# yu45020/Text_Segmentation_Image_Inpainting

Measured on NVIDIA H100. Metric: PartialConv UNet 512x512 images/sec (fwd+bwd), higher is better.
Workload: dtype bf16

## Files before the change

### text_segmentation_image_inpainting_b200/csrc/conv_tc.cu

```cuda
#include <cuda.h>
#include <stdlib.h>
#include <string.h>

#include <algorithm>

#include "pcb_common.cuh"
#include "pcb_ptx.cuh"

namespace {

constexpr int BLOCK_M = 128;
constexpr int BLOCK_K = 64;
constexpr int A_STAGE_BYTES = BLOCK_M * 128;
constexpr int NUM_PRODUCER_THREADS = 128;
constexpr int TC_MAX_PARTS = 2;
constexpr int MMA_WARPS = 8;
constexpr int MMA_THREADS = MMA_WARPS * 32;
constexpr int acc_pitch(int block_n) { return block_n + 4; }
constexpr int acc_stage_bytes(int block_n) { return BLOCK_M * acc_pitch(block_n) * 4; }

inline int rup(int v, int m) { return (v + m - 1) / m * m; }

struct TcPart {
    const bf16 *x;
// ... 7 lines not shown
    int n, h, w, cin, cout, kh, kw, stride, pad_h, pad_w, dil, ho, wo;
    int m_total;
    int nparts, no_guard, rowpack;
    int hg;
    int ring_a, ring_b;
    int ktap;
    int ncols;
    TcPart parts[TC_MAX_PARTS];
    const float *bias; const float *msum; bf16 *y; int y_cstride;
    const bf16 *dc; int dc_cstride, dc_c8, dc_kext;
    int *abort_flag;
    int l2pf;
    int box_w, box_h, box_n, stages, use_fix;
    int wk_base, wk_row, wk_col;
    int sub, py, px, fh, fw;
    int ksplit;
    float *partial;
    double *bn_sums;
    int bn_c;
};

constexpr int STAT_SLICE = 256;
constexpr int STAT_SMEM_BYTES = MMA_WARPS * STAT_SLICE * 4 + 16;

__device__ __forceinline__ float warp_transpose_sum(float (&v)[32], int lane) {
#pragma unroll
    for (int off = 16, n = 32; off >= 1; off >>= 1, n >>= 1) {
        const bool upper = (lane & off) != 0;
#pragma unroll
        for (int i = 0; i < 16; ++i) {
            if (i < (n >> 1)) {
                const float send = upper ? v[i] : v[i + (n >> 1)];
                const float keep = upper ? v[i + (n >> 1)] : v[i];
                v[i] = keep + __shfl_xor_sync(0xffffffffu, send, off);
            }
        }
    }
    return v[0];
}

__device__ __forceinline__ uint32_t align1024(uint32_t a) { return (a + 1023u) & ~1023u; }

__device__ __forceinline__ void load_acc32(const float *src, uint32_t (&r)[32]) {
#pragma unroll
    for (int j = 0; j < 8; ++j) {
        const uint4 v = reinterpret_cast<const uint4 *>(src)[j];
        r[4 * j] = v.x; r[4 * j + 1] = v.y; r[4 * j + 2] = v.z; r[4 * j + 3] = v.w;
    }
}

template <int BLOCK_N, int MODE>
__device__ __forceinline__ void tc_epilogue(const TcParams &P, const float *acc_row, int warp, int lane, int m0, int n0, float *s_stat,
                                            int cb, int ce, int sq_off) {
                const int row = warp * 32 + lane;
                const int m = m0 + row;
                const bool rvalid = m < P.m_total;
                float inv = 0.f;
                bool hole = false;
                int en = 0, eh = 0, ew = 0;
                long long mo = m;
                if (MODE == 1 && rvalid) {
                    en = m / (P.h * P.w); const int rem = m - en * P.h * P.w; eh = rem / P.w; ew = rem - eh * P.w;
                    eh = eh * P.sub + P.py; ew = ew * P.sub + P.px;
                    mo = (static_cast<long long>(en) * P.fh + eh) * P.fw + ew;
                }
                if (MODE == 0 && rvalid && P.sub != 1) {
                    en = m / (P.ho * P.wo); const int rem = m - en * P.ho * P.wo; eh = rem / P.wo; ew = rem - eh * P.wo;
                    mo = (static_cast<long long>(en) * P.fh + eh * P.sub + P.py) * P.fw + ew * P.sub + P.px;
                }
                if (MODE == 0 && rvalid) {
                    const float s = P.msum ? P.msum[mo] : 1.f;
                    hole = (s == 0.f) && !P.no_guard;
                    inv = hole ? 0.f : 1.0f / s;
                }
                if (P.partial != nullptr) {
    #pragma unroll 1
                    for (int c0 = cb; c0 < ce; c0 += 32) {
                        uint32_t r[32];
                        load_acc32(acc_row + c0, r);
                        if (rvalid) {
                            float *dst = P.partial + static_cast<long long>(m) * P.ncols + n0 + c0;
    #pragma unroll
                            for (int j = 0; j < 32; ++j) atomicAdd(dst + j, __uint_as_float(r[j]));
                        }
                    }
                    return;
                }
    #pragma unroll 1
                for (int c0 = cb; c0 < ce; c0 += 32) {
                    uint32_t r[32];
                    load_acc32(acc_row + c0, r);
                    const int col = n0 + c0;
                    bf16 *orow = nullptr;
                    int nstore = 0;
                    float scale = inv;
                    if (MODE == 0) {
                        if (rvalid && col < P.y_cstride) { orow = P.y + mo * P.y_cstride + col; nstore = min(32, P.y_cstride - col); }
                    } else {
                        scale = 1.f;
                        for (int p = 0; p < P.nparts; ++p) {
                            const TcPart &pt = P.parts[p];
                            const int local = col - pt.koff;
                            if (local >= 0 && local < pt.kext && pt.dx != nullptr && local < pt.c8 && rvalid) {
                                orow = pt.dx + mo * pt.dx_cstride + local;
                                nstore = min(32, pt.c8 - local);
                                if (pt.mask != nullptr)
                                    scale = pt.mask[(static_cast<long long>(en) * (P.fh >> pt.mup) + (eh >> pt.mup)) * (P.fw >> pt.mup) + (ew >> pt.mup)] ? 1.f : 0.f;
                            }
                        }
                    }
                    const bool stats = (MODE == 0) && (s_stat != nullptr);
                    if (__any_sync(0xffffffffu, nstore > 0) || stats) {
                        uint4 o[4];
                        __nv_bfloat162 *ob = reinterpret_cast<__nv_bfloat162 *>(o);
                        float bl = 0.f;
                        const bool has_bias = (MODE == 0) && (P.bias != nullptr);
                        if (has_bias && col + lane < P.cout) bl = P.bias[col + lane];
                        const bool edge = (MODE == 0) && (col + 32 > P.cout);
    #pragma unroll
                        for (int j = 0; j < 16; ++j) {
                            float a = __uint_as_float(r[2 * j]), b = __uint_as_float(r[2 * j + 1]);
                            if (MODE == 0) {
                                const float b0 = has_bias ? __shfl_sync(0xffffffffu, bl, 2 * j) : 0.f;
                                const float b1 = has_bias ? __shfl_sync(0xffffffffu, bl, 2 * j + 1) : 0.f;
                                a = hole ? 0.f : fmaf(a, scale, b0);
                                b = hole ? 0.f : fmaf(b, scale, b1);
                                if (edge) {
                                    if (col + 2 * j >= P.cout) a = 0.f;
                                    if (col + 2 * j + 1 >= P.cout) b = 0.f;
                                }
// ... 32 lines not shown
        const int co = n0 + c0 + lane;
        if (co < P.bn_c) {
            atomicAdd(P.bn_sums + co, static_cast<double>(s_stat[c0 - cb + lane]));
            atomicAdd(P.bn_sums + P.bn_c + co, static_cast<double>(s_stat[sq_off + c0 - cb + lane]));
        }
        s_stat[c0 - cb + lane] = 0.f; s_stat[sq_off + c0 - cb + lane] = 0.f;
    }
    __syncwarp();
}

template <int BLOCK_N>
struct EpiRole {
    static constexpr int HN = (BLOCK_N >= 64) ? BLOCK_N / 2 : BLOCK_N;
    int q, half, cb, ce;
    __device__ __forceinline__ explicit EpiRole(int e) {
        q = 2 * (e >> 2) + (e & 1);
        half = (e & 3) >> 1;
        cb = half * HN;
        ce = (cb + HN <= BLOCK_N) ? cb + HN : cb;
    }
    __device__ __forceinline__ int slice() const { return half * 4 + q; }
};

template <int BLOCK_N, int MODE>
__device__ __forceinline__ void mma_epilogue(const TcParams &P, const float (&acc)[BLOCK_N / 2], float *stage, int e, int lane, int m0, int n0,
                                             float *s_stat) {
    constexpr int PITCH = acc_pitch(BLOCK_N);
    const int g = e >> 2;
    const int r0 = 64 * g + 16 * (e & 3) + (lane >> 2), c0 = 2 * (lane & 3);
#pragma unroll
    for (int i = 0; i < BLOCK_N / 2; i += 2) {
        const int row = r0 + 8 * ((i >> 1) & 1), col = 8 * (i >> 2) + c0;
        *reinterpret_cast<float2 *>(stage + row * PITCH + col) = make_float2(acc[i], acc[i + 1]);
    }
    ptx::named_sync(1 + g, 128);
    const EpiRole<BLOCK_N> R(e);
    tc_epilogue<BLOCK_N, MODE>(P, stage + (R.q * 32 + lane) * PITCH, R.q, lane, m0, n0, s_stat, R.cb, R.ce, 128);
    ptx::named_sync(1 + g, 128);
}

template <int BLOCK_N>
__device__ __forceinline__ void tc_stats_final(const TcParams &P, const float *stat_base, int e, int lane, int stat_n0) {
    constexpr int HN = EpiRole<BLOCK_N>::HN;
    for (int col = e * 32 + lane; col < BLOCK_N; col += MMA_THREADS) {
        const int co = stat_n0 + col;
        if (co < P.bn_c) {
            const int h = col / HN, lc = col - h * HN;
            float a = 0.f, q = 0.f;
#pragma unroll
            for (int w4 = 0; w4 < 4; ++w4) { a += stat_base[(h * 4 + w4) * STAT_SLICE + lc]; q += stat_base[(h * 4 + w4) * STAT_SLICE + 128 + lc]; }
            atomicAdd(P.bn_sums + co, static_cast<double>(a));
            atomicAdd(P.bn_sums + P.bn_c + co, static_cast<double>(q));
        }
    }
}

template <int R> __device__ __forceinline__ void zero_acc(float (&a)[R]) {
#pragma unroll
    for (int i = 0; i < R; ++i) a[i] = 0.f;
}

constexpr int HALO_MAX_HG = 12;
constexpr int PERSIST_THREADS = 4 * 32 + MMA_THREADS + 32;
constexpr int MAX_RING = 8;

template <int BLOCK_N, int MODE, bool HALO>
__global__ void __launch_bounds__(PERSIST_THREADS, 1)
pconv_tc_persistent_kernel(const __grid_constant__ TcParams P, const __grid_constant__ CUtensorMap tmap_w) {
    constexpr int B_STAGE_BYTES = BLOCK_N * 128;
    extern __shared__ uint8_t smem_raw[];
    const uint32_t smem_base = align1024(ptx::smem_u32(smem_raw));
    const int SA = P.ring_a, SB = P.ring_b;
    const int HG = P.hg;
// ... 335 lines not shown
                    } else {
                        const uint64_t da = ptx::make_smem_desc(sA + sa * A_STAGE + g * a_rows, 16, 1024);
#pragma unroll
                        for (int k = 0; k < BLOCK_K / 16; ++k)
                            ptx::wgmma_bf16<BLOCK_N, 0, 0>(acc, da + 2 * k, db + 2 * k);
                    }
                    ptx::wgmma_commit();
                }
                ptx::wgmma_wait<0>();
                ptx::wgmma_fence_regs(acc);
                if (leader) {
                    for (int tc = 0; tc < nB; ++tc) ptx::mbar_arrive(bar_empty_b + 8 * ((sb0 + tc) % SB));
                    ptx::mbar_arrive(bar_empty_a + 8 * sa);
                }
            }
            if (dead) { stat_n0 = -1; break; }
            mma_epilogue<BLOCK_N, MODE>(P, acc, acc_stage, e, lane, m0, n0, my_stat);
        }
        if (my_stat && stat_n0 >= 0) tc_stats_flush<BLOCK_N>(P, my_stat, lane, stat_n0, R.cb, R.ce, 128);
    }
}


constexpr int TMA_THREADS = MMA_THREADS + 5 * 32;

template <int BLOCK_N, int MODE, bool HALO>
__global__ void __launch_bounds__(TMA_THREADS, 1)
pconv_tc_tma_kernel(const __grid_constant__ TcParams P, const __grid_constant__ CUtensorMap tmap_w,
                    const __grid_constant__ CUtensorMap tmap_a0, const __grid_constant__ CUtensorMap tmap_a1) {
    constexpr uint32_t B_BYTES = BLOCK_N * 128;
    extern __shared__ uint8_t smem_raw[];
    const uint32_t smem_base = align1024(ptx::smem_u32(smem_raw));
    const int S = P.stages;
    const int nB = HALO ? P.kw : 1;
    const int hx = HALO ? (P.kw - 1) * P.dil : 0;
    const uint32_t A_BYTES = static_cast<uint32_t>(BLOCK_M + hx) * 128u;
    const uint32_t A_ROOM = (A_BYTES + 1023u) & ~1023u;
    const uint32_t STAGE = A_ROOM + nB * B_BYTES;
    const uint32_t STAGE_TX = A_BYTES + nB * B_BYTES;
    const uint32_t sBar = smem_base + S * STAGE;
    const uint32_t bar_full = sBar, bar_fixed = sBar + 8 * MAX_RING, bar_empty = sBar + 16 * MAX_RING;
    const uint32_t s_stat_addr = sBar + 24 * MAX_RING;
    const uint32_t s_acc = (s_stat_addr + STAT_SMEM_BYTES + 15u) & ~15u;
    uint8_t *smem_gen = smem_raw + (smem_base - ptx::smem_u32(smem_raw));

    const int warp = __shfl_sync(0xffffffffu, threadIdx.x >> 5, 0), lane = threadIdx.x & 31;
    const int np = (MODE == 0) ? P.nparts : 1;
    const int n_tiles = P.ncols / BLOCK_N;
    const int KS = P.ksplit;
    const int m_tiles = (P.m_total + BLOCK_M - 1) / BLOCK_M;
    const int num_tiles = m_tiles * n_tiles * KS;
    const int tile0 = static_cast<int>(blockIdx.x), tstep = static_cast<int>(gridDim.x);
    auto m0_of = [&](int mt) -> int { return mt * BLOCK_M; };
    const bool fix = (MODE == 0) && P.use_fix;
    const int kwi = HALO ? 1 : P.kw;

    auto tile_active = [&](int n0) -> bool {
        if (MODE == 0) return true;
        for (int p = 0; p < P.nparts; ++p)
            if (P.parts[p].dx && n0 < P.parts[p].koff + P.parts[p].kext && n0 + BLOCK_N > P.parts[p].koff) return true;
        return false;
    };

    if (threadIdx.x == 0) {
        for (int s = 0; s < MAX_RING; ++s) {
            ptx::mbar_init(bar_full + 8 * s, 1); ptx::mbar_init(bar_fixed + 8 * s, 4); ptx::mbar_init(bar_empty + 8 * s, 2);
        }
        ptx::fence_mbar_init();
    }
    if (warp == 8 && lane == 0) { ptx::prefetch_tmap(&tmap_w); ptx::prefetch_tmap(&tmap_a0); if (np > 1) ptx::prefetch_tmap(&tmap_a1); }
    __syncthreads();

    float *s_stat = nullptr;
    int stat_n0 = -1;
    if (warp == 8) {
        int s = 0;
        uint32_t ph = 1;
        const int plane = (MODE == 0) ? P.ho * P.wo : P.h * P.w;
        const int pwid = (MODE == 0) ? P.wo : P.w;
        const int kext0 = (MODE == 0) ? P.parts[0].kext : P.dc_kext, kext1 = (MODE == 0 && np > 1) ? P.parts[1].kext : 0;
        const int dstep = (MODE == 0) ? P.dil : -P.dil;
        const int row_k = P.wk_row, col_k = P.wk_col;
        bool dead = false;
        for (int tile = tile0; tile < num_tiles && !dead; tile += tstep) {
            const int sp = tile % KS, mn = tile / KS;
            const int m0 = m0_of(mn / n_tiles), n0 = (mn % n_tiles) * BLOCK_N;
            if (!tile_active(n0)) continue;
            const int img = m0 / plane, rem = m0 - img * plane;
            const int oy = rem / pwid, ox = rem - oy * pwid;
            const int x_org = (MODE == 0) ? ox * P.stride - P.pad_w : (HALO ? ox + P.pad_w - hx : ox + P.pad_w);
            const int y_org = (MODE == 0) ? oy * P.stride - P.pad_h : oy + P.pad_h;
            int nx_org = 0, ny_org = 0, nimg = -1;
            if (P.l2pf && tile + tstep < num_tiles) {
                const int nmn = (tile + tstep) / KS;
                const int nm0 = m0_of(nmn / n_tiles);
                if (nm0 != m0) {
                    nimg = nm0 / plane;
                    const int nrem = nm0 - nimg * plane, noy = nrem / pwid, nox = nrem - noy * pwid;
// ... 24 lines not shown
                            __syncwarp();
                            if (++s == S) { s = 0; ph ^= 1; }
                        }
                        if (dead) break;
                    }
                }
        }
    } else if (warp < MMA_WARPS) {
        const int e = warp, g = warp >> 2;
        const bool leader = (threadIdx.x & 127) == 0;
        const uint32_t ready = fix ? bar_fixed : bar_full;
        const uint64_t desc_a0 = ptx::make_smem_desc(smem_base + g * 64 * 128, 16, 1024);
        const uint64_t desc_b0 = ptx::make_smem_desc(smem_base + A_ROOM, 16, 1024);
        const uint32_t stage16 = STAGE >> 4;
        const int shift0 = (HALO && MODE == 1) ? hx * 8 : 0;
        const int dshift = HALO ? ((MODE == 1) ? -P.dil * 8 : P.dil * 8) : 0;
        const int rows_a = P.kh * kwi;
        int nb0, nb1 = 0, kl0, kl1 = 4;
        {
            const int kext = (MODE == 0) ? P.parts[0].kext : P.dc_kext, c8 = (MODE == 0) ? P.parts[0].c8 : P.dc_c8;
            nb0 = kext / BLOCK_K; kl0 = min(4, (c8 - (nb0 - 1) * BLOCK_K + 15) >> 4);
            if (MODE == 0 && np > 1) { nb1 = P.parts[1].kext / BLOCK_K; kl1 = min(4, (P.parts[1].c8 - (nb1 - 1) * BLOCK_K + 15) >> 4); }
        }
        const EpiRole<BLOCK_N> R(e);
        s_stat = (MODE == 0 && P.bn_sums != nullptr && P.partial == nullptr)
                     ? reinterpret_cast<float *>(smem_gen + (s_stat_addr - smem_base)) + R.slice() * STAT_SLICE : nullptr;
        if (s_stat) {
            for (int i = lane; i < STAT_SLICE; i += 32) s_stat[i] = 0.f;
            __syncwarp();
        }
        float *acc_stage = reinterpret_cast<float *>(smem_gen + (s_acc - smem_base));
        int s = 0;
        uint32_t ph = 0;
        bool dead = false;
        for (int tile = tile0; tile < num_tiles && !dead; tile += tstep) {
            const int sp = tile % KS, mn = tile / KS;
            const int m0 = m0_of(mn / n_tiles), n0 = (mn % n_tiles) * BLOCK_N;
            if (!tile_active(n0)) continue;
            if (s_stat && n0 != stat_n0) {
                if (stat_n0 >= 0) tc_stats_flush<BLOCK_N>(P, s_stat, lane, stat_n0, R.cb, R.ce, 128);
                stat_n0 = n0;
            }
            float acc[BLOCK_N / 2];
            zero_acc(acc);
            int held = -1;
            for (int r = 0; r < rows_a && !dead; ++r) {
#pragma unroll
                for (int p = 0; p < TC_MAX_PARTS; ++p) {
                    const int nbp = (p == 0) ? nb0 : nb1, klast = (p == 0) ? kl0 : kl1;
                    const int gb0 = (p == 0) ? 0 : nb0;
                    for (int cb = 0; cb < nbp; ++cb) {
                        if (KS > 1 && (gb0 + cb) % KS != sp) continue;
                        if (!__all_sync(0xffffffffu, ptx::mbar_wait(ready + 8 * s, ph, P.abort_flag, 124))) { dead = true; break; }
                        uint64_t da = desc_a0 + static_cast<uint64_t>(s * stage16 + shift0), db = desc_b0 + static_cast<uint64_t>(s * stage16);
                        const int ksteps = (cb + 1 < nbp) ? 4 : klast;
                        ptx::wgmma_fence();
                        for (int tc = 0; tc < nB; ++tc, da += dshift, db += B_BYTES >> 4) {
                            if (ksteps == 4) {
#pragma unroll
                                for (int k = 0; k < 4; ++k) ptx::wgmma_bf16<BLOCK_N, 0, 0>(acc, da + 2 * k, db + 2 * k);
                            } else {
                                for (int k = 0; k < ksteps; ++k) ptx::wgmma_bf16<BLOCK_N, 0, 0>(acc, da + 2 * k, db + 2 * k);
                            }
                        }
                        ptx::wgmma_commit();
                        ptx::wgmma_wait<1>();
                        if (held >= 0 && leader) ptx::mbar_arrive(bar_empty + 8 * held);
                        held = s;
                        if (++s == S) { s = 0; ph ^= 1; }
                    }
                    if (dead) break;
                }
            }
            ptx::wgmma_wait<0>();
            ptx::wgmma_fence_regs(acc);
            if (held >= 0 && leader) ptx::mbar_arrive(bar_empty + 8 * held);
            if (dead) { stat_n0 = -1; break; }
            mma_epilogue<BLOCK_N, MODE>(P, acc, acc_stage, e, lane, m0, n0, s_stat);
        }
    } else if (warp > 8) {
        if (fix) {
            const int t = (warp - 9) * 32 + lane;
            int s = 0;
            uint32_t ph = 0;
            bool dead = false;
            if (!HALO) {
                uint64_t wnext[TC_MAX_PARTS];
                auto load_words = [&](int tl) {
#pragma unroll
                    for (int p = 0; p < TC_MAX_PARTS; ++p) {
                        wnext[p] = 0ull;
                        const int m = m0_of(tl / KS / n_tiles) + t;
                        if (fix && p < P.nparts && tl < num_tiles && m < P.m_total) wnext[p] = __ldg(P.parts[p].tapmask + m);
                    }
                };
                load_words(tile0);
                for (int tile = tile0; tile < num_tiles && !dead; tile += tstep) {
                    const int sp = tile % KS;
                    uint64_t wcur[TC_MAX_PARTS];
#pragma unroll
                    for (int p = 0; p < TC_MAX_PARTS; ++p) wcur[p] = wnext[p];
// ... 75 lines not shown
#pragma unroll
                                        for (int k = 0; k < 8; ++k) r[k] = z;
                                    }
                                    if (h1) {
                                        uint4 *r = reinterpret_cast<uint4 *>(smem_gen + s * STAGE + (t + 128) * 128);
#pragma unroll
                                        for (int k = 0; k < 8; ++k) r[k] = z;
                                    }
                                    ptx::fence_proxy_async_smem();
                                }
                                __syncwarp();
                                if (lane == 0) ptx::mbar_arrive(bar_fixed + 8 * s);
                                if (++s == S) { s = 0; ph ^= 1; }
                            }
                            if (dead) break;
                        }
                    }
                }
            }
        }
    }

    __syncthreads();
    if (s_stat != nullptr && stat_n0 >= 0) tc_stats_final<BLOCK_N>(P, s_stat - EpiRole<BLOCK_N>(warp).slice() * STAT_SLICE, warp, lane, stat_n0);
}


constexpr int SP_MAX_ITEMS = 40;
struct SpItem { int part, dx, dy, wk, nb, wk_step, shift0, dshift; };
struct SpTable {
    int n_items;
    int step[TC_MAX_PARTS];
    int es[TC_MAX_PARTS];
    int ph[TC_MAX_PARTS], pw[TC_MAX_PARTS];
    int arows[TC_MAX_PARTS];
    int rows_max;
    SpItem it[SP_MAX_ITEMS];
};

template <int BLOCK_N, int MODE>
__global__ void __launch_bounds__(TMA_THREADS, 1)
pconv_tc_sp_kernel(const __grid_constant__ TcParams P, const __grid_constant__ SpTable TB, const __grid_constant__ CUtensorMap tmap_w,
                   const __grid_constant__ CUtensorMap tmap_a0, const __grid_constant__ CUtensorMap tmap_a1) {
    constexpr uint32_t B_BYTES = BLOCK_N * 128;
    extern __shared__ uint8_t smem_raw[];
    const uint32_t smem_base = align1024(ptx::smem_u32(smem_raw));
    const int S = P.stages;
    int nb_max = 1;
    for (int i = 0; i < TB.n_items; ++i) nb_max = max(nb_max, TB.it[i].nb);
    const uint32_t A_ROOM = (static_cast<uint32_t>(TB.rows_max) * 128u + 1023u) & ~1023u;
    const uint32_t STAGE = A_ROOM + nb_max * B_BYTES;
    const uint32_t sBar = smem_base + S * STAGE;
    const uint32_t bar_full = sBar, bar_fixed = sBar + 8 * MAX_RING, bar_empty = sBar + 16 * MAX_RING;
    const uint32_t s_stat_addr = sBar + 24 * MAX_RING;
    const uint32_t s_acc = (s_stat_addr + STAT_SMEM_BYTES + 15u) & ~15u;
    uint8_t *smem_gen = smem_raw + (smem_base - ptx::smem_u32(smem_raw));

    const int warp = __shfl_sync(0xffffffffu, threadIdx.x >> 5, 0), lane = threadIdx.x & 31;
    const int n_tiles = P.ncols / BLOCK_N;
    const int m_tiles = (P.m_total + BLOCK_M - 1) / BLOCK_M;
    const int num_tiles = m_tiles * n_tiles;
    const int tile0 = static_cast<int>(blockIdx.x), tstep = static_cast<int>(gridDim.x);
    const bool fix = P.use_fix != 0;
    const int gw = (MODE == 0) ? P.wo : P.w, gh = (MODE == 0) ? P.ho : P.h;
    const int plane = gw * gh;
    int nbk[TC_MAX_PARTS], klast[TC_MAX_PARTS];
#pragma unroll
    for (int p = 0; p < TC_MAX_PARTS; ++p) {
        const int kext = (MODE == 0) ? P.parts[p].kext : P.dc_kext, c8 = (MODE == 0) ? P.parts[p].c8 : P.dc_c8;
        nbk[p] = (p < ((MODE == 0) ? P.nparts : 1)) ? kext / BLOCK_K : 0;
        klast[p] = nbk[p] ? min(4, (c8 - (nbk[p] - 1) * BLOCK_K + 15) >> 4) : 4;
    }

    if (threadIdx.x == 0) {
        for (int s = 0; s < MAX_RING; ++s) { ptx::mbar_init(bar_full + 8 * s, 1); ptx::mbar_init(bar_fixed + 8 * s, 4); ptx::mbar_init(bar_empty + 8 * s, 2); }
        ptx::fence_mbar_init();
    }
    if (warp == 8 && lane == 0) { ptx::prefetch_tmap(&tmap_w); ptx::prefetch_tmap(&tmap_a0); ptx::prefetch_tmap(&tmap_a1); }
    __syncthreads();

    float *s_stat = nullptr;
    int stat_n0 = -1;
    if (warp == 8) {
        int s = 0;
        uint32_t ph = 1;
        bool dead = false;
        for (int tile = tile0; tile < num_tiles && !dead; tile += tstep) {
            const int m0 = (tile / n_tiles) * BLOCK_M, n0 = (tile % n_tiles) * BLOCK_N;
            const int img = m0 / plane, rem = m0 - img * plane;
            const int oy = rem / gw, ox = rem - oy * gw;
            for (int i = 0; i < TB.n_items && !dead; ++i) {
                const SpItem it = TB.it[i];
                const CUtensorMap *ma = (it.part == 0) ? &tmap_a0 : &tmap_a1;
                const int x = ox * TB.step[it.part] + it.dx, y = oy * TB.step[it.part] + it.dy;
                const uint32_t a_bytes = static_cast<uint32_t>(TB.arows[it.part]) * 128u;
                for (int cb = 0; cb < nbk[it.part]; ++cb) {
                    if (!__all_sync(0xffffffffu, ptx::mbar_wait(bar_empty + 8 * s, ph, P.abort_flag, 321))) { dead = true; break; }
                    if (ptx::elect_one()) {
                        const uint32_t full = bar_full + 8 * s, dst = smem_base + s * STAGE;
                        ptx::mbar_arrive_expect_tx(full, a_bytes + it.nb * B_BYTES);
                        ptx::tma_load_4d(dst, ma, cb * BLOCK_K, x, y, img, full);
                        uint32_t bdst = dst + A_ROOM;
                        for (int tc = 0, kb = it.wk + cb * BLOCK_K; tc < it.nb; ++tc, kb += it.wk_step, bdst += B_BYTES)
                            ptx::tma_load_2d(bdst, &tmap_w, kb, n0, full);
                    }
                    __syncwarp();
                    if (++s == S) { s = 0; ph ^= 1; }
                }
            }
        }
    } else if (warp < MMA_WARPS) {
        const int e = warp, g = warp >> 2;
        const bool leader = (threadIdx.x & 127) == 0;
        const uint32_t ready = fix ? bar_fixed : bar_full;
        const uint64_t desc_a0 = ptx::make_smem_desc(smem_base + g * 64 * 128, 16, 1024);
        const uint64_t desc_b0 = ptx::make_smem_desc(smem_base + A_ROOM, 16, 1024);
        const uint32_t stage16 = STAGE >> 4;
        const EpiRole<BLOCK_N> R(e);
        s_stat = (MODE == 0 && P.bn_sums != nullptr) ? reinterpret_cast<float *>(smem_gen + (s_stat_addr - smem_base)) + R.slice() * STAT_SLICE : nullptr;
        if (s_stat) {
            for (int i = lane; i < STAT_SLICE; i += 32) s_stat[i] = 0.f;
            __syncwarp();
        }
        float *acc_stage = reinterpret_cast<float *>(smem_gen + (s_acc - smem_base));
        int s = 0;
        uint32_t ph = 0;
        bool dead = false;
        for (int tile = tile0; tile < num_tiles && !dead; tile += tstep) {
            const int m0 = (tile / n_tiles) * BLOCK_M, n0 = (tile % n_tiles) * BLOCK_N;
            if (s_stat && n0 != stat_n0) {
                if (stat_n0 >= 0) tc_stats_flush<BLOCK_N>(P, s_stat, lane, stat_n0, R.cb, R.ce, 128);
                stat_n0 = n0;
            }
            float acc[BLOCK_N / 2];
            zero_acc(acc);
            int held = -1;
            for (int i = 0; i < TB.n_items && !dead; ++i) {
                const SpItem it = TB.it[i];
                for (int cb = 0; cb < nbk[it.part]; ++cb) {
                    if (!__all_sync(0xffffffffu, ptx::mbar_wait(ready + 8 * s, ph, P.abort_flag, 324))) { dead = true; break; }
                    uint64_t da = desc_a0 + static_cast<uint64_t>(s * stage16 + it.shift0), db = desc_b0 + static_cast<uint64_t>(s * stage16);
                    const int ksteps = (cb + 1 < nbk[it.part]) ? 4 : klast[it.part];
                    ptx::wgmma_fence();
                    for (int tc = 0; tc < it.nb; ++tc, da += it.dshift, db += B_BYTES >> 4)
                        for (int k = 0; k < ksteps; ++k) ptx::wgmma_bf16<BLOCK_N, 0, 0>(acc, da + 2 * k, db + 2 * k);
                    ptx::wgmma_commit();
                    ptx::wgmma_wait<1>();
                    if (held >= 0 && leader) ptx::mbar_arrive(bar_empty + 8 * held);
                    held = s;
                    if (++s == S) { s = 0; ph ^= 1; }
                }
            }
            ptx::wgmma_wait<0>();
            ptx::wgmma_fence_regs(acc);
            if (held >= 0 && leader) ptx::mbar_arrive(bar_empty + 8 * held);
            if (dead) { stat_n0 = -1; break; }
            mma_epilogue<BLOCK_N, MODE>(P, acc, acc_stage, e, lane, m0, n0, s_stat);
        }
    } else if (warp > 8) {
        if (fix) {
            const int t = (warp - 9) * 32 + lane;
            int s = 0;
            uint32_t ph = 0;
            bool dead = false;
            auto load_bits = [&](int tl, uint64_t &b0, uint64_t &b1) {
                b0 = b1 = 0ull;
                if (tl >= num_tiles) return;
                const int m0 = (tl / n_tiles) * BLOCK_M;
                const int img = m0 / plane, rem = m0 - img * plane;
                const int oy = rem / gw, ox = rem - oy * gw;
                for (int i = 0; i < TB.n_items; ++i) {
                    const SpItem it = TB.it[i];
                    const uint8_t *mk = P.parts[it.part].mask;
                    if (mk == nullptr) continue;
                    const int pwid = TB.pw[it.part], phei = TB.ph[it.part], es = TB.es[it.part];
                    const int hrows = TB.arows[it.part] - BLOCK_M;
                    const int x0 = ox * TB.step[it.part] + it.dx, y0 = oy * TB.step[it.part] + it.dy;
                    int tx, ty, tn;
                    if (hrows > 0 || (P.box_h == 1 && P.box_n == 1)) { tx = t; ty = 0; tn = 0; }
                    else { tx = t % P.box_w; ty = (t / P.box_w) % P.box_h; tn = t / (P.box_w * P.box_h); }
// ... 21 lines not shown
                            const uint4 z = make_uint4(0u, 0u, 0u, 0u);
                            if (h0) {
                                uint4 *r = reinterpret_cast<uint4 *>(smem_gen + s * STAGE + t * 128);
#pragma unroll
                                for (int k = 0; k < 8; ++k) r[k] = z;
                            }
                            if (h1) {
                                uint4 *r = reinterpret_cast<uint4 *>(smem_gen + s * STAGE + (t + 128) * 128);
#pragma unroll
                                for (int k = 0; k < 8; ++k) r[k] = z;
                            }
                            ptx::fence_proxy_async_smem();
                        }
                        __syncwarp();
                        if (lane == 0) ptx::mbar_arrive(bar_fixed + 8 * s);
                        if (++s == S) { s = 0; ph ^= 1; }
                    }
                }
            }
        }
    }

    __syncthreads();
    if (s_stat != nullptr && stat_n0 >= 0) tc_stats_final<BLOCK_N>(P, s_stat - EpiRole<BLOCK_N>(warp).slice() * STAT_SLICE, warp, lane, stat_n0);
}

__global__ void upsample_part_kernel(const bf16 *__restrict__ src, int cstride, int c8, long long pixels_src, int hs, int ws, bf16 *__restrict__ dst) {
    const int chunks = c8 >> 3;
    const long long total = pixels_src * chunks;
    for (long long i = blockIdx.x * static_cast<long long>(blockDim.x) + threadIdx.x; i < total; i += static_cast<long long>(gridDim.x) * blockDim.x) {
        const int ch = static_cast<int>(i % chunks);
        const long long pix = i / chunks;
        const int x = static_cast<int>(pix % ws);
        const long long t = pix / ws;
        const int y = static_cast<int>(t % hs);
        const long long n = t / hs;
        const uint4 v = __ldg(reinterpret_cast<const uint4 *>(src + pix * cstride + ch * 8));
        bf16 *d = dst + ((n * (2 * hs) + 2 * y) * (2ll * ws) + 2 * x) * c8 + ch * 8;
        uint4 *d0 = reinterpret_cast<uint4 *>(d), *d1 = reinterpret_cast<uint4 *>(d + 2ll * ws * c8);
        d0[0] = v; *reinterpret_cast<uint4 *>(d + c8) = v;
        d1[0] = v; *reinterpret_cast<uint4 *>(d + 2ll * ws * c8 + c8) = v;
    }
}

struct WgParams {
    int n, h, w, cin, cout, kh, kw, stride, pad_h, pad_w, dil, ho, wo;
    int m_total;
// ... 780 lines not shown
}

bool tma_dgrad_s2_ok(const pcb_conv *c) {
    if (getenv("PCB_DISABLE_TMA") || getenv("PCB_DISABLE_TMA_S2") || is_rowpack(c)) return false;
    if (c->stride != 2 || c->dil != 1 || c->kh < 2 || c->kw < 2 || ((c->h | c->w) & 1) || c->ho != c->h / 2 || c->wo != c->w / 2) return false;
    int bw, bh, bn;
    return tile_box(c->w / 2, c->h / 2, &bw, &bh, &bn);
}

size_t up_bytes(const pcb_conv *c, int p) {
    return (static_cast<size_t>(c->n) * c->h * c->w * rup(c->parts[p].c, 8) * 2 + 255) / 256 * 256;
}
size_t tapmask_bytes(const pcb_conv *c) {
    return (static_cast<size_t>(c->nparts) * c->n * c->ho * c->wo * sizeof(uint64_t) + 255) / 256 * 256;
}

template <int BLOCK_N, int MODE, bool HALO>
int launch_tma_n(TcParams &P, const CUtensorMap &tw, const CUtensorMap &ta0, const CUtensorMap &ta1, cudaStream_t st) {
    const int nb = HALO ? P.kw : 1;
    const size_t a_room = (static_cast<size_t>(BLOCK_M + (HALO ? (P.kw - 1) * P.dil : 0)) * 128 + 1023) / 1024 * 1024;
    const size_t stage = a_room + static_cast<size_t>(nb) * BLOCK_N * 128;
    P.stages = static_cast<int>(std::min<size_t>(MAX_RING, (RING_BUDGET - acc_stage_bytes(BLOCK_N)) / stage));
    PCB_CHECK(P.stages >= 2, "TMA-fed conv: stage of %zu bytes does not fit twice", stage);
    const size_t smem = 1024 + P.stages * stage + 24 * MAX_RING + 16 + STAT_SMEM_BYTES + acc_stage_bytes(BLOCK_N);
    auto kern = pconv_tc_tma_kernel<BLOCK_N, MODE, HALO>;
    PCB_SMEM_OPT_IN(kern, MAX_SMEM);
    if (P.ksplit < 1) P.ksplit = 1;
    const int m_tiles = (P.m_total + BLOCK_M - 1) / BLOCK_M;
    const int num_tiles = m_tiles * (P.ncols / BLOCK_N) * P.ksplit;
    const int grid = std::min(num_tiles, pcb_num_sms());
    kern<<<grid, TMA_THREADS, smem, st>>>(P, tw, ta0, ta1);
    PCB_LAUNCH_CHECK();
    return 0;
}

template <int MODE>
int launch_tma(TcParams &P, const CUtensorMap &tw, const CUtensorMap &ta0, const CUtensorMap &ta1, int bn, bool halo, cudaStream_t st) {
    if (halo) {
        if (bn == 128) return launch_tma_n<128, MODE, true>(P, tw, ta0, ta1, st);
        if (bn == 64) return launch_tma_n<64, MODE, true>(P, tw, ta0, ta1, st);
        return launch_tma_n<32, MODE, true>(P, tw, ta0, ta1, st);
    }
    if (bn == 128) return launch_tma_n<128, MODE, false>(P, tw, ta0, ta1, st);
    if (bn == 64) return launch_tma_n<64, MODE, false>(P, tw, ta0, ta1, st);
    return launch_tma_n<32, MODE, false>(P, tw, ta0, ta1, st);
}

// ... 177 lines not shown
    }
    for (int q = 0; q < 2; ++q)
        for (int e = 0; e < 4; ++e) { W.ybits[q][e] = S.ay.tapbits[q][e]; W.xbits[q][e] = S.ax.tapbits[q][e]; }
    if (S.fwd) {
        sp_weight_prepare_kernel<<<dim3(c->cout, slot), 128, 0, st>>>(w_master, W, w_f, w_d);
        PCB_LAUNCH_CHECK();
    } else if (S.dgrad) {
        sp_weight_dg_kernel<<<dim3(W.c_u, S.net_total), 128, 0, st>>>(w_master, W, w_d);
        PCB_LAUNCH_CHECK();
    }
    return 0;
}

int sp_bn(int cols, long long m_total) { return std::min(pick_bn(cols, m_total), 64); }

template <int BLOCK_N, int MODE>
int launch_sp_n(TcParams &P, const SpTable &TB, const CUtensorMap &tw, const CUtensorMap &ta0, const CUtensorMap &ta1, cudaStream_t st) {
    int nb_max = 1;
    for (int i = 0; i < TB.n_items; ++i) nb_max = std::max(nb_max, TB.it[i].nb);
    const size_t a_room = (static_cast<size_t>(TB.rows_max) * 128 + 1023) / 1024 * 1024;
    const size_t stage = a_room + static_cast<size_t>(nb_max) * BLOCK_N * 128;
    P.stages = static_cast<int>(std::min<size_t>(MAX_RING, (RING_BUDGET - acc_stage_bytes(BLOCK_N)) / stage));
    PCB_CHECK(P.stages >= 2, "sub-pixel conv: stage of %zu bytes does not fit twice", stage);
    const size_t smem = 1024 + P.stages * stage + 24 * MAX_RING + 16 + STAT_SMEM_BYTES + acc_stage_bytes(BLOCK_N);
    auto kern = pconv_tc_sp_kernel<BLOCK_N, MODE>;
    PCB_SMEM_OPT_IN(kern, MAX_SMEM);
    const int num_tiles = ((P.m_total + BLOCK_M - 1) / BLOCK_M) * (P.ncols / BLOCK_N);
    const int grid = std::min(num_tiles, pcb_num_sms());
    kern<<<grid, TMA_THREADS, smem, st>>>(P, TB, tw, ta0, ta1);
    PCB_LAUNCH_CHECK();
    return 0;
}

template <int MODE>
int launch_sp(TcParams &P, const SpTable &TB, const CUtensorMap &tw, const CUtensorMap &ta0, const CUtensorMap &ta1, int bn, cudaStream_t st) {
    if (bn == 64) return launch_sp_n<64, MODE>(P, TB, tw, ta0, ta1, st);
    return launch_sp_n<32, MODE>(P, TB, tw, ta0, ta1, st);
}

struct ClassStreams4 { cudaStream_t aux[3]; cudaEvent_t ev_fork, ev_join[3]; bool ready; };
int class_streams(ClassStreams4 **out) {
    static thread_local ClassStreams4 cs_all[PCB_MAX_DEVICES] = {};
    ClassStreams4 &CS = cs_all[pcb_cur_device()];
    if (!CS.ready) {
        for (int i = 0; i < 3; ++i) {
            PCB_CUDA(cudaStreamCreateWithFlags(&CS.aux[i], cudaStreamNonBlocking));
            PCB_CUDA(cudaEventCreateWithFlags(&CS.ev_join[i], cudaEventDisableTiming));
// ... 590 lines not shown
```

Before: 854.2.

## Add dedicated epilogue warps fed by mbarrier handoff in TMA conv kernels

```diff
diff --git a/text_segmentation_image_inpainting_b200/csrc/conv_tc.cu b/text_segmentation_image_inpainting_b200/csrc/conv_tc.cu
--- a/text_segmentation_image_inpainting_b200/csrc/conv_tc.cu
+++ b/text_segmentation_image_inpainting_b200/csrc/conv_tc.cu
@@ -53,6 +53,8 @@
 
 constexpr int STAT_SLICE = 256;
 constexpr int STAT_SMEM_BYTES = MMA_WARPS * STAT_SLICE * 4 + 16;
+constexpr int EPI_WARPS = 4;
+constexpr int EPI_STAT_SMEM_BYTES = EPI_WARPS * STAT_SLICE * 4;
 
 __device__ __forceinline__ float warp_transpose_sum(float (&v)[32], int lane) {
 #pragma unroll
@@ -80,30 +82,55 @@
     }
 }
 
+struct EpiRow {
+    long long mo;
+    int m;
+    bool rvalid, hole;
+    float inv;
+    float dscale[TC_MAX_PARTS];
+};
+
+template <int MODE>
+__device__ __forceinline__ EpiRow tc_epi_row(const TcParams &P, int m) {
+    EpiRow er;
+    er.m = m;
+    er.rvalid = m < P.m_total;
+    er.inv = 0.f;
+    er.hole = false;
+    er.mo = m;
+    int en = 0, eh = 0, ew = 0;
+    if (MODE == 1 && er.rvalid) {
+        en = m / (P.h * P.w); const int rem = m - en * P.h * P.w; eh = rem / P.w; ew = rem - eh * P.w;
+        eh = eh * P.sub + P.py; ew = ew * P.sub + P.px;
+        er.mo = (static_cast<long long>(en) * P.fh + eh) * P.fw + ew;
+    }
+    if (MODE == 0 && er.rvalid && P.sub != 1) {
+        en = m / (P.ho * P.wo); const int rem = m - en * P.ho * P.wo; eh = rem / P.wo; ew = rem - eh * P.wo;
+        er.mo = (static_cast<long long>(en) * P.fh + eh * P.sub + P.py) * P.fw + ew * P.sub + P.px;
+    }
+    if (MODE == 0 && er.rvalid) {
+        const float s = P.msum ? P.msum[er.mo] : 1.f;
+        er.hole = (s == 0.f) && !P.no_guard;
+        er.inv = er.hole ? 0.f : 1.0f / s;
+    }
+#pragma unroll
+    for (int p = 0; p < TC_MAX_PARTS; ++p) {
+        er.dscale[p] = 1.f;
+        if (MODE == 1 && p < P.nparts) {
+            const TcPart &pt = P.parts[p];
+            if (er.rvalid && pt.dx != nullptr && pt.mask != nullptr)
+                er.dscale[p] = pt.mask[(static_cast<long long>(en) * (P.fh >> pt.mup) + (eh >> pt.mup)) * (P.fw >> pt.mup) + (ew >> pt.mup)] ? 1.f : 0.f;
+        }
+    }
+    return er;
+}
+
 template <int BLOCK_N, int MODE>
-__device__ __forceinline__ void tc_epilogue(const TcParams &P, const float *acc_row, int warp, int lane, int m0, int n0, float *s_stat,
+__device__ __forceinline__ void tc_epilogue(const TcParams &P, const EpiRow &er, const float *acc_row, int lane, int n0, float *s_stat,
                                             int cb, int ce, int sq_off) {
-                const int row = warp * 32 + lane;
-                const int m = m0 + row;
-                const bool rvalid = m < P.m_total;
-                float inv = 0.f;
-                bool hole = false;
-                int en = 0, eh = 0, ew = 0;
-                long long mo = m;
-                if (MODE == 1 && rvalid) {
-                    en = m / (P.h * P.w); const int rem = m - en * P.h * P.w; eh = rem / P.w; ew = rem - eh * P.w;
-                    eh = eh * P.sub + P.py; ew = ew * P.sub + P.px;
-                    mo = (static_cast<long long>(en) * P.fh + eh) * P.fw + ew;
-                }
-                if (MODE == 0 && rvalid && P.sub != 1) {
-                    en = m / (P.ho * P.wo); const int rem = m - en * P.ho * P.wo; eh = rem / P.wo; ew = rem - eh * P.wo;
-                    mo = (static_cast<long long>(en) * P.fh + eh * P.sub + P.py) * P.fw + ew * P.sub + P.px;
-                }
-                if (MODE == 0 && rvalid) {
-                    const float s = P.msum ? P.msum[mo] : 1.f;
-                    hole = (s == 0.f) && !P.no_guard;
-                    inv = hole ? 0.f : 1.0f / s;
-                }
+                const int m = er.m;
+                const bool rvalid = er.rvalid, hole = er.hole;
+                const long long mo = er.mo;
                 if (P.partial != nullptr) {
     #pragma unroll 1
                     for (int c0 = cb; c0 < ce; c0 += 32) {
@@ -124,19 +151,20 @@
                     const int col = n0 + c0;
                     bf16 *orow = nullptr;
                     int nstore = 0;
-                    float scale = inv;
+                    float scale = er.inv;
                     if (MODE == 0) {
                         if (rvalid && col < P.y_cstride) { orow = P.y + mo * P.y_cstride + col; nstore = min(32, P.y_cstride - col); }
                     } else {
                         scale = 1.f;
-                        for (int p = 0; p < P.nparts; ++p) {
+#pragma unroll
+                        for (int p = 0; p < TC_MAX_PARTS; ++p) {
+                            if (p >= P.nparts) break;
                             const TcPart &pt = P.parts[p];
                             const int local = col - pt.koff;
                             if (local >= 0 && local < pt.kext && pt.dx != nullptr && local < pt.c8 && rvalid) {
                                 orow = pt.dx + mo * pt.dx_cstride + local;
                                 nstore = min(32, pt.c8 - local);
-                                if (pt.mask != nullptr)
-                                    scale = pt.mask[(static_cast<long long>(en) * (P.fh >> pt.mup) + (eh >> pt.mup)) * (P.fw >> pt.mup) + (ew >> pt.mup)] ? 1.f : 0.f;
+                                scale = er.dscale[p];
                             }
                         }
                     }
@@ -215,33 +243,38 @@
     __device__ __forceinline__ int slice() const { return half * 4 + q; }
 };
 
+template <int BLOCK_N>
+__device__ __forceinline__ void stage_acc(const float (&acc)[BLOCK_N / 2], float *stage, int e, int lane) {
+    constexpr int PITCH = acc_pitch(BLOCK_N);
+    const int r0 = 64 * (e >> 2) + 16 * (e & 3) + (lane >> 2), c0 = 2 * (lane & 3);
+#pragma unroll
+    for (int i = 0; i < BLOCK_N / 2; i += 2) {
+        const int row = r0 + 8 * ((i >> 1) & 1), col = 8 * (i >> 2) + c0;
+        *reinterpret_cast<float2 *>(stage + row * PITCH + col) = make_float2(acc[i], acc[i + 1]);
+    }
+}
+
 template <int BLOCK_N, int MODE>
 __device__ __forceinline__ void mma_epilogue(const TcParams &P, const float (&acc)[BLOCK_N / 2], float *stage, int e, int lane, int m0, int n0,
                                              float *s_stat) {
     constexpr int PITCH = acc_pitch(BLOCK_N);
     const int g = e >> 2;
-    const int r0 = 64 * g + 16 * (e & 3) + (lane >> 2), c0 = 2 * (lane & 3);
-#pragma unroll
-    for (int i = 0; i < BLOCK_N / 2; i += 2) {
-        const int row = r0 + 8 * ((i >> 1) & 1), col = 8 * (i >> 2) + c0;
-        *reinterpret_cast<float2 *>(stage + row * PITCH + col) = make_float2(acc[i], acc[i + 1]);
-    }
+    stage_acc<BLOCK_N>(acc, stage, e, lane);
     ptx::named_sync(1 + g, 128);
     const EpiRole<BLOCK_N> R(e);
-    tc_epilogue<BLOCK_N, MODE>(P, stage + (R.q * 32 + lane) * PITCH, R.q, lane, m0, n0, s_stat, R.cb, R.ce, 128);
+    const EpiRow er = tc_epi_row<MODE>(P, m0 + R.q * 32 + lane);
+    tc_epilogue<BLOCK_N, MODE>(P, er, stage + (R.q * 32 + lane) * PITCH, lane, n0, s_stat, R.cb, R.ce, 128);
     ptx::named_sync(1 + g, 128);
 }
 
 template <int BLOCK_N>
-__device__ __forceinline__ void tc_stats_final(const TcParams &P, const float *stat_base, int e, int lane, int stat_n0) {
-    constexpr int HN = EpiRole<BLOCK_N>::HN;
-    for (int col = e * 32 + lane; col < BLOCK_N; col += MMA_THREADS) {
+__device__ __forceinline__ void tc_stats_final(const TcParams &P, const float *stat_base, int w, int lane, int stat_n0) {
+    for (int col = w * 32 + lane; col < BLOCK_N; col += EPI_WARPS * 32) {
         const int co = stat_n0 + col;
         if (co < P.bn_c) {
-            const int h = col / HN, lc = col - h * HN;
             float a = 0.f, q = 0.f;
 #pragma unroll
-            for (int w4 = 0; w4 < 4; ++w4) { a += stat_base[(h * 4 + w4) * STAT_SLICE + lc]; q += stat_base[(h * 4 + w4) * STAT_SLICE + 128 + lc]; }
+            for (int w4 = 0; w4 < EPI_WARPS; ++w4) { a += stat_base[w4 * STAT_SLICE + col]; q += stat_base[w4 * STAT_SLICE + 128 + col]; }
             atomicAdd(P.bn_sums + co, static_cast<double>(a));
             atomicAdd(P.bn_sums + P.bn_c + co, static_cast<double>(q));
         }
@@ -623,7 +656,49 @@
 }
 
 
-constexpr int TMA_THREADS = MMA_THREADS + 5 * 32;
+constexpr int EPI_WARP0 = MMA_WARPS + 5;
+constexpr int TMA_THREADS = (EPI_WARP0 + EPI_WARPS) * 32;
+
+constexpr size_t TMA_BAR_BYTES = 24 * MAX_RING + 16;
+
+template <int BLOCK_N, int MODE, typename TileFn>
+__device__ __forceinline__ void tma_epilogue_warps(const TcParams &P, int tile0, int tstep, int num_tiles, TileFn tile_origin,
+                                                   const float *acc_stage, uint32_t acc_full, uint32_t acc_empty, float *s_stat,
+                                                   int &stat_n0, int w, int lane, int code) {
+    constexpr int PITCH = acc_pitch(BLOCK_N);
+    const float *acc_row = acc_stage + (w * 32 + lane) * PITCH;
+    if (s_stat) {
+        for (int i = lane; i < STAT_SLICE; i += 32) s_stat[i] = 0.f;
+        __syncwarp();
+    }
+    uint32_t ph = 0;
+    for (int tile = tile0; tile < num_tiles; tile += tstep) {
+        int m0, n0;
+        tile_origin(tile, m0, n0);
+        if (n0 < 0) continue;
+        if (s_stat && n0 != stat_n0) {
+            if (stat_n0 >= 0) tc_stats_flush<BLOCK_N>(P, s_stat, lane, stat_n0, 0, BLOCK_N, 128);
+            stat_n0 = n0;
+        }
+        const EpiRow er = tc_epi_row<MODE>(P, m0 + w * 32 + lane);
+        if (!__all_sync(0xffffffffu, ptx::mbar_wait(acc_full, ph, P.abort_flag, code))) { stat_n0 = -1; return; }
+        ph ^= 1;
+        tc_epilogue<BLOCK_N, MODE>(P, er, acc_row, lane, n0, s_stat, 0, BLOCK_N, 128);
+        __syncwarp();
+        if (lane == 0) ptx::mbar_arrive(acc_empty);
+    }
+}
+
+template <int BLOCK_N>
+__device__ __forceinline__ bool tma_stage_tile(const TcParams &P, const float (&acc)[BLOCK_N / 2], float *acc_stage, uint32_t acc_full,
+                                               uint32_t acc_empty, uint32_t &ph, int e, int lane, int code) {
+    if (!__all_sync(0xffffffffu, ptx::mbar_wait(acc_empty, ph, P.abort_flag, code))) return false;
+    ph ^= 1;
+    stage_acc<BLOCK_N>(acc, acc_stage, e, lane);
+    __syncwarp();
+    if (lane == 0) ptx::mbar_arrive(acc_full);
+    return true;
+}
 
 template <int BLOCK_N, int MODE, bool HALO>
 __global__ void __launch_bounds__(TMA_THREADS, 1)
@@ -641,8 +716,9 @@
     const uint32_t STAGE_TX = A_BYTES + nB * B_BYTES;
     const uint32_t sBar = smem_base + S * STAGE;
     const uint32_t bar_full = sBar, bar_fixed = sBar + 8 * MAX_RING, bar_empty = sBar + 16 * MAX_RING;
-    const uint32_t s_stat_addr = sBar + 24 * MAX_RING;
-    const uint32_t s_acc = (s_stat_addr + STAT_SMEM_BYTES + 15u) & ~15u;
+    const uint32_t acc_full = sBar + 24 * MAX_RING, acc_empty = acc_full + 8;
+    const uint32_t s_stat_addr = sBar + TMA_BAR_BYTES;
+    const uint32_t s_acc = s_stat_addr + EPI_STAT_SMEM_BYTES;
     uint8_t *smem_gen = smem_raw + (smem_base - ptx::smem_u32(smem_raw));
 
     const int warp = __shfl_sync(0xffffffffu, threadIdx.x >> 5, 0), lane = threadIdx.x & 31;
@@ -667,6 +743,7 @@
         for (int s = 0; s < MAX_RING; ++s) {
             ptx::mbar_init(bar_full + 8 * s, 1); ptx::mbar_init(bar_fixed + 8 * s, 4); ptx::mbar_init(bar_empty + 8 * s, 2);
         }
+        ptx::mbar_init(acc_full, MMA_WARPS); ptx::mbar_init(acc_empty, EPI_WARPS);
         ptx::fence_mbar_init();
     }
     if (warp == 8 && lane == 0) { ptx::prefetch_tmap(&tmap_w); ptx::prefetch_tmap(&tmap_a0); if (np > 1) ptx::prefetch_tmap(&tmap_a1); }
@@ -674,7 +751,18 @@
 
     float *s_stat = nullptr;
     int stat_n0 = -1;
-    if (warp == 8) {
+    float *acc_stage = reinterpret_cast<float *>(smem_gen + (s_acc - smem_base));
+    if (warp >= EPI_WARP0) {
+        const int w = warp - EPI_WARP0;
+        s_stat = (MODE == 0 && P.bn_sums != nullptr && P.partial == nullptr)
+                     ? reinterpret_cast<float *>(smem_gen + (s_stat_addr - smem_base)) + w * STAT_SLICE : nullptr;
+        auto origin = [&](int tile, int &m0, int &n0) {
+            const int mn = tile / KS;
+            m0 = m0_of(mn / n_tiles); n0 = (mn % n_tiles) * BLOCK_N;
+            if (!tile_active(n0)) n0 = -1;
+        };
+        tma_epilogue_warps<BLOCK_N, MODE>(P, tile0, tstep, num_tiles, origin, acc_stage, acc_full, acc_empty, s_stat, stat_n0, w, lane, 126);
+    } else if (warp == 8) {
         int s = 0;
         uint32_t ph = 1;
         const int plane = (MODE == 0) ? P.ho * P.wo : P.h * P.w;
@@ -745,25 +833,13 @@
             nb0 = kext / BLOCK_K; kl0 = min(4, (c8 - (nb0 - 1) * BLOCK_K + 15) >> 4);
             if (MODE == 0 && np > 1) { nb1 = P.parts[1].kext / BLOCK_K; kl1 = min(4, (P.parts[1].c8 - (nb1 - 1) * BLOCK_K + 15) >> 4); }
         }
-        const EpiRole<BLOCK_N> R(e);
-        s_stat = (MODE == 0 && P.bn_sums != nullptr && P.partial == nullptr)
-                     ? reinterpret_cast<float *>(smem_gen + (s_stat_addr - smem_base)) + R.slice() * STAT_SLICE : nullptr;
-        if (s_stat) {
-            for (int i = lane; i < STAT_SLICE; i += 32) s_stat[i] = 0.f;
-            __syncwarp();
-        }
-        float *acc_stage = reinterpret_cast<float *>(smem_gen + (s_acc - smem_base));
         int s = 0;
-        uint32_t ph = 0;
+        uint32_t ph = 0, aph = 1;
         bool dead = false;
         for (int tile = tile0; tile < num_tiles && !dead; tile += tstep) {
             const int sp = tile % KS, mn = tile / KS;
-            const int m0 = m0_of(mn / n_tiles), n0 = (mn % n_tiles) * BLOCK_N;
+            const int n0 = (mn % n_tiles) * BLOCK_N;
             if (!tile_active(n0)) continue;
-            if (s_stat && n0 != stat_n0) {
-                if (stat_n0 >= 0) tc_stats_flush<BLOCK_N>(P, s_stat, lane, stat_n0, R.cb, R.ce, 128);
-                stat_n0 = n0;
-            }
             float acc[BLOCK_N / 2];
             zero_acc(acc);
             int held = -1;
@@ -798,8 +874,8 @@
             ptx::wgmma_wait<0>();
             ptx::wgmma_fence_regs(acc);
             if (held >= 0 && leader) ptx::mbar_arrive(bar_empty + 8 * held);
-            if (dead) { stat_n0 = -1; break; }
-            mma_epilogue<BLOCK_N, MODE>(P, acc, acc_stage, e, lane, m0, n0, s_stat);
+            if (dead) break;
+            if (!tma_stage_tile<BLOCK_N>(P, acc, acc_stage, acc_full, acc_empty, aph, e, lane, 125)) break;
         }
     } else if (warp > 8) {
         if (fix) {
@@ -921,7 +997,7 @@
     }
 
     __syncthreads();
-    if (s_stat != nullptr && stat_n0 >= 0) tc_stats_final<BLOCK_N>(P, s_stat - EpiRole<BLOCK_N>(warp).slice() * STAT_SLICE, warp, lane, stat_n0);
+    if (s_stat != nullptr && stat_n0 >= 0) tc_stats_final<BLOCK_N>(P, s_stat - (warp - EPI_WARP0) * STAT_SLICE, warp - EPI_WARP0, lane, stat_n0);
 }
 
 
@@ -951,8 +1027,9 @@
     const uint32_t STAGE = A_ROOM + nb_max * B_BYTES;
     const uint32_t sBar = smem_base + S * STAGE;
     const uint32_t bar_full = sBar, bar_fixed = sBar + 8 * MAX_RING, bar_empty = sBar + 16 * MAX_RING;
-    const uint32_t s_stat_addr = sBar + 24 * MAX_RING;
-    const uint32_t s_acc = (s_stat_addr + STAT_SMEM_BYTES + 15u) & ~15u;
+    const uint32_t acc_full = sBar + 24 * MAX_RING, acc_empty = acc_full + 8;
+    const uint32_t s_stat_addr = sBar + TMA_BAR_BYTES;
+    const uint32_t s_acc = s_stat_addr + EPI_STAT_SMEM_BYTES;
     uint8_t *smem_gen = smem_raw + (smem_base - ptx::smem_u32(smem_raw));
 
     const int warp = __shfl_sync(0xffffffffu, threadIdx.x >> 5, 0), lane = threadIdx.x & 31;
@@ -973,6 +1050,7 @@
 
     if (threadIdx.x == 0) {
         for (int s = 0; s < MAX_RING; ++s) { ptx::mbar_init(bar_full + 8 * s, 1); ptx::mbar_init(bar_fixed + 8 * s, 4); ptx::mbar_init(bar_empty + 8 * s, 2); }
+        ptx::mbar_init(acc_full, MMA_WARPS); ptx::mbar_init(acc_empty, EPI_WARPS);
         ptx::fence_mbar_init();
     }
     if (warp == 8 && lane == 0) { ptx::prefetch_tmap(&tmap_w); ptx::prefetch_tmap(&tmap_a0); ptx::prefetch_tmap(&tmap_a1); }
@@ -980,7 +1058,13 @@
 
     float *s_stat = nullptr;
     int stat_n0 = -1;
-    if (warp == 8) {
+    float *acc_stage = reinterpret_cast<float *>(smem_gen + (s_acc - smem_base));
+    if (warp >= EPI_WARP0) {
+        const int w = warp - EPI_WARP0;
+        s_stat = (MODE == 0 && P.bn_sums != nullptr) ? reinterpret_cast<float *>(smem_gen + (s_stat_addr - smem_base)) + w * STAT_SLICE : nullptr;
+        auto origin = [&](int tile, int &m0, int &n0) { m0 = (tile / n_tiles) * BLOCK_M; n0 = (tile % n_tiles) * BLOCK_N; };
+        tma_epilogue_warps<BLOCK_N, MODE>(P, tile0, tstep, num_tiles, origin, acc_stage, acc_full, acc_empty, s_stat, stat_n0, w, lane, 326);
+    } else if (warp == 8) {
         int s = 0;
         uint32_t ph = 1;
         bool dead = false;
@@ -1015,22 +1099,10 @@
         const uint64_t desc_a0 = ptx::make_smem_desc(smem_base + g * 64 * 128, 16, 1024);
         const uint64_t desc_b0 = ptx::make_smem_desc(smem_base + A_ROOM, 16, 1024);
         const uint32_t stage16 = STAGE >> 4;
-        const EpiRole<BLOCK_N> R(e);
-        s_stat = (MODE == 0 && P.bn_sums != nullptr) ? reinterpret_cast<float *>(smem_gen + (s_stat_addr - smem_base)) + R.slice() * STAT_SLICE : nullptr;
-        if (s_stat) {
-            for (int i = lane; i < STAT_SLICE; i += 32) s_stat[i] = 0.f;
-            __syncwarp();
-        }
-        float *acc_stage = reinterpret_cast<float *>(smem_gen + (s_acc - smem_base));
         int s = 0;
-        uint32_t ph = 0;
+        uint32_t ph = 0, aph = 1;
         bool dead = false;
         for (int tile = tile0; tile < num_tiles && !dead; tile += tstep) {
-            const int m0 = (tile / n_tiles) * BLOCK_M, n0 = (tile % n_tiles) * BLOCK_N;
-            if (s_stat && n0 != stat_n0) {
-                if (stat_n0 >= 0) tc_stats_flush<BLOCK_N>(P, s_stat, lane, stat_n0, R.cb, R.ce, 128);
-                stat_n0 = n0;
-            }
             float acc[BLOCK_N / 2];
             zero_acc(acc);
             int held = -1;
@@ -1053,8 +1125,8 @@
             ptx::wgmma_wait<0>();
             ptx::wgmma_fence_regs(acc);
             if (held >= 0 && leader) ptx::mbar_arrive(bar_empty + 8 * held);
-            if (dead) { stat_n0 = -1; break; }
-            mma_epilogue<BLOCK_N, MODE>(P, acc, acc_stage, e, lane, m0, n0, s_stat);
+            if (dead) break;
+            if (!tma_stage_tile<BLOCK_N>(P, acc, acc_stage, acc_full, acc_empty, aph, e, lane, 325)) break;
         }
     } else if (warp > 8) {
         if (fix) {
@@ -1122,7 +1194,7 @@
     }
 
     __syncthreads();
-    if (s_stat != nullptr && stat_n0 >= 0) tc_stats_final<BLOCK_N>(P, s_stat - EpiRole<BLOCK_N>(warp).slice() * STAT_SLICE, warp, lane, stat_n0);
+    if (s_stat != nullptr && stat_n0 >= 0) tc_stats_final<BLOCK_N>(P, s_stat - (warp - EPI_WARP0) * STAT_SLICE, warp - EPI_WARP0, lane, stat_n0);
 }
 
 __global__ void upsample_part_kernel(const bf16 *__restrict__ src, int cstride, int c8, long long pixels_src, int hs, int ws, bf16 *__restrict__ dst) {
@@ -1949,7 +2021,7 @@
     const size_t stage = a_room + static_cast<size_t>(nb) * BLOCK_N * 128;
     P.stages = static_cast<int>(std::min<size_t>(MAX_RING, (RING_BUDGET - acc_stage_bytes(BLOCK_N)) / stage));
     PCB_CHECK(P.stages >= 2, "TMA-fed conv: stage of %zu bytes does not fit twice", stage);
-    const size_t smem = 1024 + P.stages * stage + 24 * MAX_RING + 16 + STAT_SMEM_BYTES + acc_stage_bytes(BLOCK_N);
+    const size_t smem = 1024 + P.stages * stage + TMA_BAR_BYTES + EPI_STAT_SMEM_BYTES + acc_stage_bytes(BLOCK_N);
     auto kern = pconv_tc_tma_kernel<BLOCK_N, MODE, HALO>;
     PCB_SMEM_OPT_IN(kern, MAX_SMEM);
     if (P.ksplit < 1) P.ksplit = 1;
@@ -2173,7 +2245,7 @@
     const size_t stage = a_room + static_cast<size_t>(nb_max) * BLOCK_N * 128;
     P.stages = static_cast<int>(std::min<size_t>(MAX_RING, (RING_BUDGET - acc_stage_bytes(BLOCK_N)) / stage));
     PCB_CHECK(P.stages >= 2, "sub-pixel conv: stage of %zu bytes does not fit twice", stage);
-    const size_t smem = 1024 + P.stages * stage + 24 * MAX_RING + 16 + STAT_SMEM_BYTES + acc_stage_bytes(BLOCK_N);
+    const size_t smem = 1024 + P.stages * stage + TMA_BAR_BYTES + EPI_STAT_SMEM_BYTES + acc_stage_bytes(BLOCK_N);
     auto kern = pconv_tc_sp_kernel<BLOCK_N, MODE>;
     PCB_SMEM_OPT_IN(kern, MAX_SMEM);
     const int num_tiles = ((P.m_total + BLOCK_M - 1) / BLOCK_M) * (P.ncols / BLOCK_N);
```

Result: faster. 882.3 (median of 6 runs) (+3.3%).
